# ThomasZiegler/RS-aware-differential-SfM

Measured on AMD Instinct MI355X. Metric: Mpixels/sec RS depth+pose solve, 1280x720 pair, higher is better.
Workload: dtype f64

## Files before the change

### include/rsdsfm.h

```cpp
#ifndef RSDSFM_H
#define RSDSFM_H

#include <stddef.h>
#include <stdint.h>

#ifdef __cplusplus
extern "C" {
#endif

#define RSDSFM_OK 0
#define RSDSFM_ERR_INVALID (-1)
#define RSDSFM_ERR_HIP (-2)
#define RSDSFM_ERR_NO_DEVICE (-3)
#define RSDSFM_ERR_NUMERIC (-4)
#define RSDSFM_ERR_PENDING (-5)
#define RSDSFM_ERR_PEER (-6)

#define RSDSFM_DEPTH_CLOSED_FORM 0
#define RSDSFM_DEPTH_CERES_LM 1

#define RSDSFM_K_COMPAT 0
#define RSDSFM_K_FIXED 1

#define RSDSFM_FLOW_COMPAT_RANK 0
// ... 152 lines not shown
    int32_t rows, cols;
    double fx, fy, cx, cy, gamma;
    double* d_depth_map_colmajor;
    double* d_R_rows9_or_null;
    double* d_t_rows3_or_null;
    uint64_t seed;
} rsdsfm_frame_job;
int rsdsfm_solve_frames_dev(rsdsfm_ctx* ctx, const rsdsfm_frame_job* jobs, int32_t count, const rsdsfm_frame_params* params,
                            rsdsfm_frame_result* results);
int rsdsfm_set_sequence_lanes(rsdsfm_ctx* ctx, int32_t lanes);
int rsdsfm_set_frame_side_flatten(rsdsfm_ctx* ctx, int mode);
int rsdsfm_set_frame_tail(rsdsfm_ctx* ctx, int mode);
int rsdsfm_set_frame_handoff(rsdsfm_ctx* ctx, int mode);
int rsdsfm_set_frame_predict(rsdsfm_ctx* ctx, int mode);
int rsdsfm_lma_predict_stats(rsdsfm_ctx* ctx, int64_t* hypotheses, int64_t* ended_where_predicted);
int rsdsfm_ransac_dev(rsdsfm_ctx* ctx, const double* d_q2n, const double* d_u2n, const double* d_alpha_n,
                      const double* d_alpha_k_n, int64_t n, int use_alpha_k, int32_t iterations, double tolerance,
                      const int32_t* samples_9xT_or_null, uint64_t seed, int depth_mode, int k_sign_mode,
                      rsdsfm_ransac_out* out);
int rsdsfm_refine_dev(rsdsfm_ctx* ctx, const double* d_flow2n, int64_t n_flow, int64_t m, const double* d_inliers_3m,
                      const double* d_alpha_m, const double* d_alpha_k_m, const int64_t* d_inlier_idx_or_null,
                      const double v_in[3], const double w_in[3], double k_in, int const_acceleration,
                      int flow_index_mode, double* d_inliers_out_3m, double v_out[3], double w_out[3], double* k_out,
                      rsdsfm_lm_summary* summary_or_null);
int rsdsfm_estimate_inverse_depths_batch_dev(rsdsfm_ctx* const* ctxs, int32_t count, const double* const* d_q2n,
                                             const double* const* d_u2n, const int64_t* n, const double* v_count_x3,
                                             const double* w_count_x3, const double* k_count, const double* const* d_alpha_n,
                                             const double* const* d_alpha_k_n, double* const* d_inv_depth_n);
int rsdsfm_depth_lm_batch_launch_dev(rsdsfm_ctx* const* ctxs, int32_t count, const double* const* d_q2n, const double* const* d_u2n,
                                     const int64_t* n, const double* v_count_x3, const double* w_count_x3, const double* k_count,
// ... 143 lines not shown
```

### rs-aware-differential-sfm_amd/__init__.py

```python
import contextlib
import ctypes as C
import os
import sys

import numpy as np

from . import dist, pipeline, synth

_HERE = os.path.dirname(os.path.abspath(__file__))
LIB_PATH = os.environ.get("RSDSFM_LIB") or os.path.join(_HERE, "librsdsfm_hip.so")
LIB_PATH_FUSED = os.path.join(_HERE, "librsdsfm_hip_fused.so")
HEADER_PATH = os.path.join(os.path.dirname(_HERE), "include", "rsdsfm.h")

OK = 0
ERR_PENDING = -5
DEPTH_CLOSED_FORM, DEPTH_CERES_LM = 0, 1
K_COMPAT, K_FIXED = 0, 1
FLOW_COMPAT_RANK, FLOW_GATHERED = 0, 1
REFINE_TRACE_COLS = 8
TRACE_REJECTED, TRACE_ACCEPTED, TRACE_INVALID, TRACE_PARAMETER_TOL, TRACE_FUNCTION_TOL, TRACE_ACCEPTED_GRADIENT_TOL = 0.0, 1.0, 2.0, 3.0, 4.0, 5.0
TERMINATION = {0: "gradient", 1: "parameter", 2: "function", 3: "max_iter", 4: "failure", 5: "min_radius"}

_libs = {}

# ... 491 lines not shown

    def set_sequence_lanes(self, lanes):
        self._check(self.lib.rsdsfm_set_sequence_lanes(self._ctx, C.c_int32(int(lanes))), "rsdsfm_set_sequence_lanes")

    def set_frame_side_flatten(self, on):
        self._check(self.lib.rsdsfm_set_frame_side_flatten(self._ctx, int(on)), "rsdsfm_set_frame_side_flatten")

    def set_frame_tail(self, mode):
        self._check(self.lib.rsdsfm_set_frame_tail(self._ctx, int(mode)), "rsdsfm_set_frame_tail")

    def set_frame_handoff(self, mode):
        self._check(self.lib.rsdsfm_set_frame_handoff(self._ctx, int(mode)), "rsdsfm_set_frame_handoff")

    def set_frame_predict(self, mode):
        self._check(self.lib.rsdsfm_set_frame_predict(self._ctx, int(mode)), "rsdsfm_set_frame_predict")

    def prepared_frames_solve(self, jobs, trials=50, tol=0.05, use_acceleration_mode=False, use_refinement=True, depth_mode=DEPTH_CERES_LM,
                              k_sign_mode=K_COMPAT, flow_threshold=1e-10, flow_index_mode=FLOW_COMPAT_RANK, use_global_shutter_mode=False):
        n = len(jobs)
        arr = (FrameJob * n)()
        for a, j in zip(arr, jobs):
            K = j["K"]
            a.d_flow_img, a.rows, a.cols = int(j["d_flow_img"]), int(j["rows"]), int(j["cols"])
            a.fx, a.fy, a.cx, a.cy, a.gamma = float(K[0]), float(K[1]), float(K[2]), float(K[3]), float(j["gamma"])
            a.d_depth_map, a.d_R, a.d_t = int(j["d_depth_map"]), int(j.get("d_R") or 0) or None, int(j.get("d_t") or 0) or None
        prm = FrameParams(int(trials), int(use_acceleration_mode), int(use_refinement), int(depth_mode), int(k_sign_mode),
                          int(flow_index_mode), int(use_global_shutter_mode), 0, float(tol), float(flow_threshold), 0)
        res = (FrameResult * n)()
        fn, ctx, check = self.lib.rsdsfm_solve_frames_dev, self._ctx, self._check

# ... 2053 lines not shown
```

### rs-aware-differential-sfm_amd/csrc/frame_host.hip

```cpp
#include <stdlib.h>
#include <string.h>

#include <atomic>

#include <algorithm>
#include <new>

#include "rsdsfm_internal.hpp"
#include "sequence_host.hpp"

namespace rsdsfm {

static std::atomic<int> g_frames_in_flight[64];
int frames_in_flight(const Ctx* c) { return g_frames_in_flight[c->device & 63].load(std::memory_order_relaxed); }

int alpha_ones_launch(Ctx* c, double* d_alpha, int64_t n);
int flatten_device(Ctx* c, const double* d_img, int32_t rows, int32_t cols, int32_t col0, double fx, double fy, double cx, double cy, double gamma,
                   double thr, double* d_q, double* d_u, double* d_alpha, double* d_alpha_k, int64_t* n_out);

struct FrameRun {
    rsdsfm_frame_job job;
    rsdsfm_frame_params prm;
    size_t N = 0;
    int64_t n = 0;
// ... 376 lines not shown
int rsdsfm_set_frame_handoff(rsdsfm_ctx* ctx, int mode) {
    if (!ctx) return RSDSFM_ERR_INVALID;
    if (mode < 0 || mode > 1) return fail(&ctx->c, RSDSFM_ERR_INVALID, "mode must be 0 (the first refinement pass gathers its inliers) or 1 (the compaction launch)");
    ctx->c.frame_handoff = mode;
    return RSDSFM_OK;
}

int rsdsfm_set_frame_predict(rsdsfm_ctx* ctx, int mode) {
    if (!ctx) return RSDSFM_ERR_INVALID;
    if (mode < 0 || mode > 2) return fail(&ctx->c, RSDSFM_ERR_INVALID, "mode must be 0 (the pixel pass fuses each hypothesis' predicted iterate), 1 (the two-iterate pass) or 2 (0 with the prediction inverted)");
    ctx->c.frame_predict = mode;
    for (rsdsfm_ctx* lane : ctx->c.lanes) lane->c.frame_predict = mode;
    return RSDSFM_OK;
}

int rsdsfm_set_frame_side_flatten(rsdsfm_ctx* ctx, int mode) {
    if (!ctx) return RSDSFM_ERR_INVALID;
    if (mode < 0 || mode > 3) return fail(&ctx->c, RSDSFM_ERR_INVALID, "mode must be 0 (flatten first), 1 (flatten on a second stream), 2 (flatten behind the minimal solver) or 3 (flatten inside the solver's launch)");
    ctx->c.frame_side_flatten = mode;
    return RSDSFM_OK;
}

}

namespace rsdsfm {

int sequence_lane_count(const Ctx* c, int count) { return std::max(1, std::min<int>(count, c->seq_lanes > 0 ? c->seq_lanes : kSequenceLanesDefault)); }

int solve_frames_run(Ctx* c, const rsdsfm_frame_job* jobs, int32_t count, const rsdsfm_frame_params* prm, rsdsfm_frame_result* results, const PairHook* hook) {
    const int L = sequence_lane_count(c, count);
// ... 8 lines not shown
        if (!c->ev_seq) RSDSFM_HIP_CHECK(c, hipEventCreateWithFlags(&c->ev_seq, hipEventDisableTiming));
        RSDSFM_HIP_CHECK(c, hipEventRecord(c->ev_seq, c->stream));
    }
    for (int l = 1; l < L; ++l) {
        Ctx* lc = lane_ctx(l);
        RSDSFM_HIP_CHECK(c, hipStreamWaitEvent(lc->stream, c->ev_seq, 0));
        lc->ransac_k0 = c->ransac_k0;
        lc->ransac_math_mode = c->ransac_math_mode;
        lc->lm_arithmetic = c->lm_arithmetic;
        lc->refine_arithmetic = c->refine_arithmetic;
        lc->lma_count_only_force = c->lma_count_only_force;
        lc->frame_side_flatten = c->frame_side_flatten;
        lc->frame_tail = c->frame_tail;
        lc->frame_handoff = c->frame_handoff;
        lc->frame_predict = c->frame_predict;
        lc->refine_stage_mode = c->refine_stage_mode;
    }
    for (int l = 0; l < L; ++l) lane_ctx(l)->refine_stage_separate = L > 1;
    int first_error = RSDSFM_OK;
    int in_flight[16];
    for (int l = 0; l < 16; ++l) in_flight[l] = -1;
    auto finish_lane = [&](int l) {
        const int i = in_flight[l];
        if (i < 0) return;
        in_flight[l] = -1;
        Ctx* lc = lane_ctx(l);
        int rc = frame_finish(lc, static_cast<FrameRun*>(lc->frame_run), &results[i]);
        if (rc != RSDSFM_OK && first_error == RSDSFM_OK) {
            first_error = rc;
            if (lc != c) c->err = "pair " + std::to_string(i) + ": " + lc->err;
// ... 63 lines not shown
```

### rs-aware-differential-sfm_amd/csrc/lma_common.hpp

```cpp
#pragma once

#include "device_math.hpp"
#include "lm_common.hpp"
#include "rsdsfm_internal.hpp"

namespace rsdsfm {

constexpr double kLmaHIrr = 1.01e-6;
constexpr double kLmaEta = 1e-11;
constexpr double kLmaMarginFloor = 128.0 * 0x1p-53;
constexpr double kLmaBand = 1e-6;
constexpr double kLmaSqrtMin = 0x1p-767;

constexpr int kLmaNC = 3;
constexpr int kLmaKP = 4;
constexpr int kLmaListCap = 1024;
constexpr int kLmaSlots = 6 + 2 * kLmaNC;
constexpr int kLmaG = 5;
constexpr int kLmaRowX0 = 8;
constexpr int kLmaRowXk = 10;
constexpr int kLmaRowScore = kLmaRowXk + 5 * kLmaKP;
constexpr int kLmaRow = kLmaRowScore + 2 * kLmaNC;

struct LmaPlan {
// ... 30 lines not shown
    int count_only;
    LmaPlan plan;
};

struct LmaPx {
    double a, ge, e0, rhos, h, g;
    bool clamped;
};

__device__ __forceinline__ double lma_max_pos(double x, double lo) {
    double r;
    asm("v_max_f64 %0, %1, %2" : "=v"(r) : "v"(x), "v"(lo));
    return r;
}
template <bool FULL = false>
__device__ __forceinline__ LmaPx lma_pixel(double x, double y, double ux, double uy, double al, double ak, const Pose& p, double two_over) {
    LmaPx o;
    const double beta = two_over * __builtin_fma(p.k, ak, al);
    const double a0 = __builtin_fma(x, p.v[2], -p.v[0]), a1 = __builtin_fma(y, p.v[2], -p.v[1]);
    const double J0 = beta * a0, J1 = beta * a1;
    const double xy = x * y, xx1 = __builtin_fma(x, x, 1.0), yy1 = __builtin_fma(y, y, 1.0);
    const double bw0 = __builtin_fma(xx1, p.w[1], __builtin_fma(-xy, p.w[0], -(y * p.w[2])));
    const double bw1 = __builtin_fma(xy, p.w[1], __builtin_fma(-yy1, p.w[0], x * p.w[2]));
    const double c0 = __builtin_fma(-beta, bw0, ux), c1 = __builtin_fma(-beta, bw1, uy);
    const double r0 = c0 + J0, r1 = c1 + J1;
    const double h = __builtin_fma(J0, J0, J1 * J1);
    double g = __builtin_fma(J0, r0, J1 * r1);
    const bool clamped = h < kLmaHIrr;
    g = g * __hiloint2double(clamped ? 0 : 0x3FF00000, 0);
    const double e0 = FULL ? g / lma_max_pos(h, kLmaHIrr) : div_core(g, lma_max_pos(h, kLmaHIrr));
    const double rhos = 1.0 - e0;
    const double s0 = __builtin_fma(rhos, J0, c0), s1 = __builtin_fma(rhos, J1, c1);
    o.a = __builtin_fma(s0, s0, s1 * s1);
    o.ge = g * e0;
    o.e0 = e0;
    o.rhos = rhos;
    o.h = h;
    o.g = g;
    o.clamped = clamped;
    return o;
}
__device__ __forceinline__ double lma_max_abs(double m, double x) {
    double r;
    asm("v_max_f64 %0, %1, |%2|" : "=v"(r) : "v"(m), "v"(x));
    return r;
}
__device__ __forceinline__ double lma_margin(const LmaPx& p, const LmaCand& cd) {
    const double t = (p.a + p.ge) + p.h;
    return __builtin_fma(t, cd.c1, cd.c1x2);
}
__device__ __forceinline__ void lma_score(const LmaPx& p, double phi2, double tol2, bool& in, double& err) {
    const double e2 = __builtin_fma(p.ge, phi2, p.a);
    in = e2 < tol2;
    err = (in && e2 >= kLmaSqrtMin) ? sqrt_core(e2) : 0.0;
}
// ... 48 lines not shown
```

### rs-aware-differential-sfm_amd/csrc/ransac_host.hip

```cpp
#include <stdio.h>
#include <stdlib.h>
#include <string.h>

#include <algorithm>
#include <vector>

#include "rsdsfm_internal.hpp"

namespace rsdsfm {

namespace {


inline uint64_t splitmix64(uint64_t& state) {
    uint64_t z = (state += 0x9E3779B97F4A7C15ULL);
    z = (z ^ (z >> 30)) * 0xBF58476D1CE4E5B9ULL;
    z = (z ^ (z >> 27)) * 0x94D049BB133111EBULL;
    return z ^ (z >> 31);
}

void sample_indices(int64_t n, int T, uint64_t seed, std::vector<int32_t>& out) {
    struct Slot {
        int64_t key;
        int32_t val;
// ... 124 lines not shown
                    R.round = 0;
                    R.pc = kPcRoundEnqueue;
                } else {
                    R.pc = kPcScore;
                }
                break;
            }
            case kPcRoundEnqueue: {
                const int b0 = R.b0, B = R.B, round = R.round;
                bool flags_via_pick = false;
                if (round > 4 * kMaxIter) return fail(c, RSDSFM_ERR_NUMERIC, "LM state machines did not terminate");
                if (R.analytic && round == 0) {
                    rc = ransac_lma_launch(c, R.d_q, R.d_u, R.d_a, R.d_ak, n, R.d_hyp + (size_t)b0 * 8, B, R.d_states + b0, R.d_partials, R.d_flags,
                                           R.d_scored + b0, R.d_tcount + b0, R.d_terr + b0, tol, R.lma_cand, 2, R.d_irr_count, R.d_irr_list, R.d_unscored,
                                           nullptr, R.core_epoch ? c->d_core_flag : nullptr, R.core_epoch, R.count_only,
                                           R.own_pass ? R.d_pred_steps + b0 : nullptr, reinterpret_cast<unsigned long long*>(c->d_core_flag + 4), c->frame_predict == 2);
                } else {
                    rc = ransac_lm_round_launch(c, R.d_q, R.d_u, R.d_a, R.d_ak, n, R.d_hyp + (size_t)b0 * 8, B, R.d_states + b0, R.d_partials, R.d_flags,
                                                R.d_scored + b0, R.d_tcount + b0, R.d_terr + b0, round, tol, R.k0, R.fused_base, R.core_math,
                                                R.core_epoch ? c->d_core_flag : nullptr, R.core_epoch, R.d_unscored);
                }
                if (rc != RSDSFM_OK) return rc;
                if (round == 0 && B == T) {
                    const PickLazy lazy = R.count_only ? PickLazy{R.d_scored, R.d_unscored, R.d_flags + 1} : PickLazy();
                    if (c->ransac_score_idle < kScoreIdleLimit) {
                        if (R.count_only) {
                            rc = ransac_pick_launch(c, R.d_tcount, R.d_terr, T, R.d_hyp, R.d_best, nullptr, R.d_flags, nullptr, 0, nullptr, 0, 0, nullptr, 0.0, lazy);
                            if (rc != RSDSFM_OK) return rc;
                        }
                        rc = ransac_score_launch(c, R.d_q, R.d_u, R.d_a, R.d_ak, n, R.d_hyp, T, R.d_states, depth_mode, tol, R.d_scored, R.d_partials,
                                                 R.d_tcount, R.d_terr, R.d_unscored, R.d_flags + 1);
// ... 417 lines not shown
```

### rs-aware-differential-sfm_amd/csrc/ransac_lma_kernels.hip

```cpp
#include <stdlib.h>

#include <algorithm>

#include "lma_common.hpp"
#include "lma_stages.hpp"
#include "rsdsfm_internal.hpp"

namespace rsdsfm {

namespace {

__device__ __forceinline__ bool is_nan_bits2(double x) {
    const uint32_t h = (uint32_t)__double2hiint(x) & 0x7FFFFFFFu;
    return h > 0x7FF00000u || (h == 0x7FF00000u && __double2loint(x) != 0);
}
__device__ __forceinline__ Pose load_pose(const double* __restrict__ hyp, int t) {
    const double* h_ = hyp + (int64_t)t * 8;
    Pose p;
    p.w[0] = h_[0], p.w[1] = h_[1], p.w[2] = h_[2];
    p.v[0] = h_[3], p.v[1] = h_[4], p.v[2] = h_[5];
    p.k = h_[6];
    return p;
}
__device__ __forceinline__ bool pose_nan(const Pose& p) {
    return is_nan_bits2(p.w[0]) || is_nan_bits2(p.w[1]) || is_nan_bits2(p.w[2]) || is_nan_bits2(p.v[0]) || is_nan_bits2(p.v[1]) || is_nan_bits2(p.v[2]) ||
           is_nan_bits2(p.k);
}

}

__device__ __forceinline__ int lma_own_index(const LmaCand& cd, int pred) { return pred == cd.steps[1] ? 1 : 0; }

template <int NC, bool ERR, bool OWN>
__device__ __forceinline__ void lma_pass_body(const double2* __restrict__ q, const double2* __restrict__ u, const double* __restrict__ alpha,
                                              const double* __restrict__ alpha_k, int64_t n, const double* __restrict__ hyp, int T, const LmaCand& cd,
                                              double* __restrict__ partials, int* __restrict__ irr_count, int* __restrict__ irr_list, int64_t chunk,
                                              unsigned long long* __restrict__ clk_probe, int clk_bid, int Tg, int nwg, const int* __restrict__ pred_steps) {
    static_assert(!OWN || NC == 1, "the own-iterate form fuses one iterate");
    __shared__ double s_part[kLB][kLmaSlots + 1];
    const int g = threadIdx.x;
    if ((int)blockIdx.x == clk_bid && g == 0) {
        clk_probe[0] = __builtin_amdgcn_s_memtime();
        clk_probe[1] = __builtin_amdgcn_s_memrealtime();
    }
    const int grp = (int)blockIdx.x / nwg, bid = (int)blockIdx.x - grp * nwg;
    const int t0 = grp * Tg, Tl = min(Tg, T - t0);
    const int P = kLB / Tg;
    const int slot = g / Tg, tl = g - slot * Tg, t = t0 + tl;
    const bool active = slot < P && tl < Tl;
    const int64_t p0 = (int64_t)bid * chunk;
    const int len = (int)min(chunk, n - p0);
    const double2* __restrict__ qb = q + p0;
    const double2* __restrict__ ub = u + p0;
    const double* __restrict__ ab = alpha + p0;
    const double* __restrict__ akb = alpha_k + p0;
    double A = 0.0, B = 0.0, C = 0.0, D = 0.0, E = 0.0, G = 0.0;
    int cnt[NC];
    double es[NC];
#pragma unroll
    for (int c = 0; c < NC; ++c) cnt[c] = 0, es[c] = 0.0;
    if (active) {
        const Pose pose = load_pose(hyp, t);
        const double two_over = 2.0 / (2.0 + pose.k);
        const double phi2_own = OWN ? (lma_own_index(cd, pred_steps[t]) ? cd.phi2[1] : cd.phi2[0]) : 0.0;
        auto pixel = [&](const PixIn& px) -> bool {
            const LmaPx v = lma_pixel(px.x, px.y, px.ux, px.uy, px.al, px.ak, pose, two_over);
            A += v.a;
            B += v.ge;
            C = __builtin_fma(v.e0, v.e0, C);
            D = __builtin_fma(v.rhos, v.rhos, D);
            E = __builtin_fma(v.rhos, v.e0, E);
            G = lma_max_abs(G, v.g);
            const double m = lma_margin(v, cd);
            bool listed = v.clamped;
#pragma unroll
            for (int c = 0; c < NC; ++c) {
                const double e2 = __builtin_fma(v.ge, OWN ? phi2_own : cd.phi2[c], v.a);
                const bool in = e2 < cd.tol2;
                listed = listed || (fabs(e2 - cd.tol2) <= m);
                cnt[c] += in ? 1 : 0;
                if (ERR) {
                    const double err = sqrt_core(lma_max_pos(e2, kLmaSqrtMin));
                    es[c] = __builtin_fma(err, __hiloint2double((in && e2 >= kLmaSqrtMin) ? 0x3FF00000 : 0, 0), es[c]);
                }
            }
            return listed;
        };
        auto push = [&](unsigned i) {
            const int pos = atomicAdd(&irr_count[t], 1);
            if (pos < kLmaListCap) irr_list[(int64_t)t * kLmaListCap + pos] = (int)(p0 + (int64_t)i);
        };
        const int rounds = len / P;
        unsigned i = (unsigned)slot;
        const unsigned uP = (unsigned)P;
        PixIn pa, pb;
        int r = 0;
        if (rounds > 0) pa = load_pix(qb, ub, ab, akb, i);
        for (; r + 1 < rounds; r += 2, i += 2 * uP) {
            pb = load_pix(qb, ub, ab, akb, i + uP);
            const bool la = pixel(pa);
            pa = load_pix(qb, ub, ab, akb, r + 2 < rounds ? i + 2 * uP : i);
            const bool lb = pixel(pb);
            if (la || lb) {
                if (la) push(i);
                if (lb) push(i + uP);
            }
        }
        if (r < rounds) {
            if (pixel(pa)) push(i);
            i += uP;
        }
        if (i < (unsigned)len && pixel(load_pix(qb, ub, ab, akb, i))) push(i);
    }
    s_part[g][0] = A, s_part[g][1] = B, s_part[g][2] = C, s_part[g][3] = D, s_part[g][4] = E, s_part[g][kLmaG] = G;
#pragma unroll
    for (int c = 0; c < kLmaNC; ++c) {
        s_part[g][6 + 2 * c] = c < NC ? (double)cnt[c < NC ? c : 0] : 0.0;
        s_part[g][7 + 2 * c] = c < NC ? es[c < NC ? c : 0] : 0.0;
    }
    __syncthreads();
    for (int o = g; o < Tl * kLmaSlots; o += kLB) {
        const int tt = o / kLmaSlots, sl = o - tt * kLmaSlots;
        double r = s_part[tt][sl];
        for (int s = 1; s < P; ++s) r = sl == kLmaG ? fmax(r, s_part[s * Tg + tt][sl]) : r + s_part[s * Tg + tt][sl];
        partials[((int64_t)(t0 + tt) * nwg + bid) * kLmaSlots + sl] = r;
    }
    if ((int)blockIdx.x == clk_bid && g == 0) {
        clk_probe[2] = __builtin_amdgcn_s_memtime();
        clk_probe[3] = __builtin_amdgcn_s_memrealtime();
    }
}

template <int NC, bool ERR>
__global__ __launch_bounds__(kLB) __attribute__((amdgpu_waves_per_eu(4, 5))) void ransac_lma_kernel(const double2* __restrict__ q, const double2* __restrict__ u, const double* __restrict__ alpha,
                                                        const double* __restrict__ alpha_k, int64_t n, const double* __restrict__ hyp, int T,
                                                        const LmaCand cd, double* __restrict__ partials, int* __restrict__ irr_count,
                                                        int* __restrict__ irr_list, int64_t chunk, unsigned long long* __restrict__ clk_probe, int clk_bid,
                                                        int Tg, int nwg) {
    lma_pass_body<NC, ERR, false>(q, u, alpha, alpha_k, n, hyp, T, cd, partials, irr_count, irr_list, chunk, clk_probe, clk_bid, Tg, nwg, nullptr);
}
template <bool ERR>
__global__ __launch_bounds__(kLB) __attribute__((amdgpu_waves_per_eu(4, 5))) void ransac_lma_own_kernel(const double2* __restrict__ q, const double2* __restrict__ u, const double* __restrict__ alpha,
                                                        const double* __restrict__ alpha_k, int64_t n, const double* __restrict__ hyp, int T,
                                                        const LmaCand cd, double* __restrict__ partials, int* __restrict__ irr_count,
                                                        int* __restrict__ irr_list, int64_t chunk, unsigned long long* __restrict__ clk_probe, int clk_bid,
                                                        int Tg, int nwg, const int* __restrict__ pred_steps) {
    lma_pass_body<1, ERR, true>(q, u, alpha, alpha_k, n, hyp, T, cd, partials, irr_count, irr_list, chunk, clk_probe, clk_bid, Tg, nwg, pred_steps);
}

__device__ __forceinline__ void lma_publish(int t, const LmScal& st, const double* hist_l, int fallback, bool scored, double count, double err,
                                            LmState* states, int* flags, int* __restrict__ scored_out, double* __restrict__ trial_count,
                                            double* __restrict__ trial_err, int* steps_hist, int* __restrict__ unscored_list, int* guard_word, bool count_only) {
    LmState* state = states + t;
    if (fallback) {
        LmScal f = {};
        f.status = 0;
        f.K = KMAX;
        f.termination = -1;
        f.rho_holds = -1;
        f.launches = 0;
        f.next_launch = 1;
        f.radius = kInitialRadius;
        f.decrease_factor = 2.0;
// ... 143 lines not shown
    }
    int64_t g = (n + (int64_t)P * 8 - 1) / ((int64_t)P * 8);
    g = std::max<int64_t>(1, std::min<int64_t>(g, (int64_t)c->num_cus * std::max(1, std::min(blocks_per_cu, 8))));
    int64_t chunk = (n + g - 1) / g;
    chunk = ((chunk + P - 1) / P) * P;
    g = std::max<int64_t>(1, (n + chunk - 1) / chunk);
    *chunk_out = chunk;
    return (int)g;
}
int64_t ransac_lma_partials_doubles(const Ctx* c, int64_t n, int batch) {
    const int64_t gmax = std::min<int64_t>((int64_t)c->num_cus * 8, std::max<int64_t>(1, (n + 7) / 8));
    return gmax * batch * kLmaSlots;
}
size_t ransac_lma_list_ints(int batch) { return (size_t)batch * kLmaListCap; }

static int lma_pass_launch(Ctx* c, const double* q, const double* u, const double* a, const double* ak, int64_t n, const double* hyp, int T,
                           const LmaCand& cd, double* partials, int* irr_count, int* irr_list, int* grid_out, unsigned long long* clk = nullptr,
                           const int* pred_steps = nullptr) {
    static int occ_tab[2][kLmaNC + 1] = {{0, 0, 0, 0}, {0, 0, 0, 0}};
    const int nc = pred_steps ? 0 : std::min(std::max(cd.nc, 1), (int)kLmaNC);
    int* occ = occ_tab[cd.count_only ? 1 : 0];
    if (occ[nc] == 0) {
        int nb = 0;
        const void* fn = pred_steps ? (cd.count_only ? reinterpret_cast<const void*>(&ransac_lma_own_kernel<false>) : reinterpret_cast<const void*>(&ransac_lma_own_kernel<true>))
                         : cd.count_only ? (nc == 1 ? reinterpret_cast<const void*>(&ransac_lma_kernel<1, false>) : nc == 2 ? reinterpret_cast<const void*>(&ransac_lma_kernel<2, false>) : reinterpret_cast<const void*>(&ransac_lma_kernel<3, false>))
                                       : (nc == 1 ? reinterpret_cast<const void*>(&ransac_lma_kernel<1, true>) : nc == 2 ? reinterpret_cast<const void*>(&ransac_lma_kernel<2, true>) : reinterpret_cast<const void*>(&ransac_lma_kernel<3, true>));
        if (hipOccupancyMaxActiveBlocksPerMultiprocessor(&nb, fn, kLB, 0) != hipSuccess || nb < 1) nb = 4;
        occ[nc] = nb;
    }
    int64_t chunk;
    static const int grid_override = getenv("RSDSFM_LMA_BLOCKS_PER_CU") ? atoi(getenv("RSDSFM_LMA_BLOCKS_PER_CU")) : 0;
    int groups = 1;
    const int Tg = ransac_lma_group_size(T, &groups);
    const int per_cu = std::max(1, (grid_override > 0 ? grid_override : occ[nc]));
    int nwg = ransac_lma_grid(c, n, Tg, &chunk, per_cu);
    if (groups > 1) {
        const int64_t cap = std::max<int64_t>(1, (int64_t)c->num_cus * std::min(per_cu, 8) / groups);
        if (nwg > cap) {
            const int P = std::max(1, kLB / Tg);
            chunk = (n + cap - 1) / cap;
            chunk = ((chunk + P - 1) / P) * P;
            nwg = (int)std::max<int64_t>(1, (n + chunk - 1) / chunk);
        }
    }
    const int grid = nwg * groups;
    *grid_out = nwg;
    const double2* q2 = reinterpret_cast<const double2*>(q);
    const double2* u2 = reinterpret_cast<const double2*>(u);
    const int clk_bid = clk ? grid / 2 : -1;
#define RSDSFM_LMA_LAUNCH(NC, ERR) \
    hipLaunchKernelGGL((ransac_lma_kernel<NC, ERR>), dim3(grid), dim3(kLB), 0, c->stream, q2, u2, a, ak, n, hyp, T, cd, partials, irr_count, irr_list, chunk, clk, clk_bid, Tg, nwg)
    if (pred_steps) {
        if (cd.count_only)
            hipLaunchKernelGGL((ransac_lma_own_kernel<false>), dim3(grid), dim3(kLB), 0, c->stream, q2, u2, a, ak, n, hyp, T, cd, partials, irr_count, irr_list, chunk, clk, clk_bid, Tg, nwg, pred_steps);
        else
            hipLaunchKernelGGL((ransac_lma_own_kernel<true>), dim3(grid), dim3(kLB), 0, c->stream, q2, u2, a, ak, n, hyp, T, cd, partials, irr_count, irr_list, chunk, clk, clk_bid, Tg, nwg, pred_steps);
    } else if (cd.count_only) {
        if (cd.nc == 1) RSDSFM_LMA_LAUNCH(1, false);
        else if (cd.nc == 2) RSDSFM_LMA_LAUNCH(2, false);
        else RSDSFM_LMA_LAUNCH(3, false);
    } else if (cd.nc == 1) RSDSFM_LMA_LAUNCH(1, true);
    else if (cd.nc == 2) RSDSFM_LMA_LAUNCH(2, true);
    else RSDSFM_LMA_LAUNCH(3, true);
#undef RSDSFM_LMA_LAUNCH
    RSDSFM_HIP_CHECK(c, hipGetLastError());
    return RSDSFM_OK;
}

int ransac_lma_launch(Ctx* c, const double* q, const double* u, const double* a, const double* ak, int64_t n, const double* hyp, int T,
                      LmState* states, double* partials, int* flags, int* scored, double* trial_count, double* trial_err, double tol,
                      const int* cand_steps, int ncand, int* irr_count, int* irr_list, int* unscored_list, int* guard_word, const int* m9_core_flag,
                      int m9_core_epoch, bool count_only, const int* pred_steps, unsigned long long* pred_stats, bool pred_discard) {
    if (T < 1 || T > kLB) return fail(c, RSDSFM_ERR_INVALID, "hypothesis batch of the analytic pass exceeds 256");
    if (pred_steps && ncand != 2) return fail(c, RSDSFM_ERR_INVALID, "the own-iterate pass chooses between two candidate iterates");
    const LmaCand cd = lma_candidates(cand_steps, ncand, tol, count_only);
    int grid = 0;
    const bool prof = c->profile && c->ev_prof[0] && c->ev_prof[1];
    if (prof) RSDSFM_HIP_CHECK(c, hipEventRecord(c->ev_prof[0], c->stream));
    int rc = lma_pass_launch(c, q, u, a, ak, n, hyp, T, cd, partials, irr_count, irr_list, &grid, prof ? c->d_clk_probe : nullptr, pred_steps);
    if (rc != RSDSFM_OK) return rc;
    if (prof) {
        RSDSFM_HIP_CHECK(c, hipEventRecord(c->ev_prof[1], c->stream));
        c->prof_pending = true;
        c->prof_what = 0;
    }
    hipLaunchKernelGGL(ransac_lma_rows_decide_kernel, dim3(T), dim3(kLB), 0, c->stream, partials, grid, T, reinterpret_cast<const double2*>(q),
                       reinterpret_cast<const double2*>(u), a, ak, n, hyp, cd, irr_count, irr_list, states, flags, scored, trial_count, trial_err,
                       unscored_list, guard_word, m9_core_flag, m9_core_epoch, pred_steps, pred_stats, pred_discard ? 1 : 0);
    RSDSFM_HIP_CHECK(c, hipGetLastError());
    return RSDSFM_OK;
}

int ransac_lma_rows_doubles() { return kLmaRow; }
int ransac_lma_rows_launch(Ctx* c, const double* q, const double* u, const double* a, const double* ak, int64_t n, const double* hyp, int T,
// ... 23 lines not shown
```

### rs-aware-differential-sfm_amd/csrc/rsdsfm_internal.hpp

```cpp
#pragma once

#include <hip/hip_runtime.h>
#include <stdint.h>

#include <functional>
#include <string>
#include <vector>

#include "../../include/rsdsfm.h"

namespace rsdsfm {

constexpr int kMaxIter = 50;
constexpr int kRefineTraceCols = RSDSFM_REFINE_TRACE_COLS;
constexpr double kInitialRadius = 1e4;
constexpr double kMaxRadius = 1e16;
constexpr double kMinRadius = 1e-32;
constexpr double kMinRelDecrease = 1e-3;
constexpr double kMinLmDiag = 1e-6;
constexpr double kMaxLmDiag = 1e32;
constexpr double kFunctionTol = 1e-6;
constexpr double kGradientTol = 1e-10;
static_assert(kGradientTol < 1.0, "the indicator encoding of the gradient-maximum slots needs kGradientTol < 1");
constexpr double kParameterTol = 1e-8;
// ... 136 lines not shown
    void* link = nullptr;
    void* fuse = nullptr;
    void* last_frame = nullptr;
    void* rectify_dense = nullptr;
    unsigned* d_claim[3] = {nullptr, nullptr, nullptr};
    size_t claim_words[3] = {0, 0, 0};
    unsigned claim_epoch[3] = {0, 0, 0};
    void* dist = nullptr;
    void* frame_run = nullptr;
    hipStream_t aux_stream = nullptr;
    hipEvent_t ev_fork = nullptr, ev_join = nullptr, ev_seq = nullptr;
    int frame_side_flatten = 3;
    int frame_tail = 0;
    int frame_handoff = 0;
    int frame_predict = 0;
    unsigned long long* d_flat_counters = nullptr;
    int seq_lanes = 0;
    int refine_stage_mode = 0;
    bool refine_stage_separate = false;
    int refine_arithmetic = 0;
    int64_t refine_rf_runs = 0, refine_rf_restarts = 0, refine_rf_resolves = 0;
    int refine_rf_last_guard = 0;
    struct RansacCache {
        uint64_t tag = 0, stage_gen = 0;
        const double *d_u = nullptr, *d_inl = nullptr, *d_alpha = nullptr, *d_alpha_k = nullptr;
        const int64_t* d_idx = nullptr;
        int64_t n = 0, m = 0;
        const void* h_u = nullptr;
        double u_probe[16] = {0};
        double inl_probe[16] = {0};
// ... 187 lines not shown
int ransac_decide_rows_launch(Ctx* c, const double* rows_all, int nranks, int T, LmState* states, int64_t n_total, int round,
                              int* flags, int* scored, double* trial_count, double* trial_err, bool core_trailer = false,
                              double* cnt_rt = nullptr, int cnt_stride = 0);
int ransac_score_rows_launch(Ctx* c, const double* q, const double* u, const double* a, const double* ak, int64_t n,
                             const double* hyp, int T, const LmState* states, int depth_mode, double tol, const int* scored,
                             double* partials, double* rows);
int ransac_score_merge_launch(Ctx* c, const double* rows_all, int nranks, int T, const int* scored, double* trial_count,
                              double* trial_err, double* cnt_rt = nullptr, int cnt_stride = 0);
void sample_indices(int64_t n, int T, uint64_t seed, int32_t* out);
int64_t ransac_lma_partials_doubles(const Ctx* c, int64_t n, int batch);
size_t ransac_lma_list_ints(int batch);
int ransac_lma_launch(Ctx* c, const double* q, const double* u, const double* a, const double* ak, int64_t n, const double* hyp, int T,
                      LmState* states, double* partials, int* flags, int* scored, double* trial_count, double* trial_err, double tol,
                      const int* cand_steps, int ncand, int* irr_count, int* irr_list, int* unscored_list, int* guard_word,
                      const int* m9_core_flag = nullptr, int m9_core_epoch = 0, bool count_only = false, const int* pred_steps = nullptr,
                      unsigned long long* pred_stats = nullptr, bool pred_discard = false);
int ransac_lma_rows_doubles();
int ransac_lma_rows_launch(Ctx* c, const double* q, const double* u, const double* a, const double* ak, int64_t n, const double* hyp, int T,
                           double* partials, double tol, const int* cand_steps, int ncand, int* irr_count, int* irr_list, double* rows);
int ransac_lma_decide_rows_launch(Ctx* c, const double* rows_all, int nranks, int64_t rank_stride, int T, int64_t n_total, const double* hyp,
                                  LmState* states, int* flags, int* scored, double* trial_count, double* trial_err, double tol, const int* cand_steps,
                                  int ncand, int* unscored_list, int* guard_word, double* cnt_rt, int cnt_stride, const int* m9_core_flag = nullptr,
                                  int m9_core_epoch = 0);
}

namespace rsdsfm {
struct RefineState {
    int32_t np, cur, iteration, invalid_run, num_successful, num_unsuccessful, termination, solve_ok;
    double p[7], pc[7], sp[7], yp[7];
    double radius, decrease_factor, cost, initial_cost, x_norm, gmax, stepsq_p;
    int64_t m;
// ... 186 lines not shown
```

Baseline: 1910.

## Stage per-pixel LMA operands in shared memory once per workgroup

Adds staged variants of the analytic LM pixel pass. Each workgroup loads a tile of pixel operands once into double-buffered LDS and shares them across all hypothesis lanes, instead of every lane loading them from global memory. When k is uniform it also precomputes the per-pixel beta and coordinate products (xy, x²+1, y²+1). By default staging is on when the hypothesis group size is at least 16. It adds block-wide barriers and more LDS use, which may lower occupancy.

```diff
diff --git a/include/rsdsfm.h b/include/rsdsfm.h
--- a/include/rsdsfm.h
+++ b/include/rsdsfm.h
@@ -190,6 +190,7 @@
 int rsdsfm_set_frame_handoff(rsdsfm_ctx* ctx, int mode);
 int rsdsfm_set_frame_predict(rsdsfm_ctx* ctx, int mode);
 int rsdsfm_lma_predict_stats(rsdsfm_ctx* ctx, int64_t* hypotheses, int64_t* ended_where_predicted);
+int rsdsfm_set_lma_operands(rsdsfm_ctx* ctx, int mode);
 int rsdsfm_ransac_dev(rsdsfm_ctx* ctx, const double* d_q2n, const double* d_u2n, const double* d_alpha_n,
                       const double* d_alpha_k_n, int64_t n, int use_alpha_k, int32_t iterations, double tolerance,
                       const int32_t* samples_9xT_or_null, uint64_t seed, int depth_mode, int k_sign_mode,
diff --git a/rs-aware-differential-sfm_amd/__init__.py b/rs-aware-differential-sfm_amd/__init__.py
--- a/rs-aware-differential-sfm_amd/__init__.py
+++ b/rs-aware-differential-sfm_amd/__init__.py
@@ -529,6 +529,9 @@
 
     def set_frame_predict(self, mode):
         self._check(self.lib.rsdsfm_set_frame_predict(self._ctx, int(mode)), "rsdsfm_set_frame_predict")
+
+    def set_lma_operands(self, mode):
+        self._check(self.lib.rsdsfm_set_lma_operands(self._ctx, int(mode)), "rsdsfm_set_lma_operands")
 
     def prepared_frames_solve(self, jobs, trials=50, tol=0.05, use_acceleration_mode=False, use_refinement=True, depth_mode=DEPTH_CERES_LM,
                               k_sign_mode=K_COMPAT, flow_threshold=1e-10, flow_index_mode=FLOW_COMPAT_RANK, use_global_shutter_mode=False):
diff --git a/rs-aware-differential-sfm_amd/csrc/frame_host.hip b/rs-aware-differential-sfm_amd/csrc/frame_host.hip
--- a/rs-aware-differential-sfm_amd/csrc/frame_host.hip
+++ b/rs-aware-differential-sfm_amd/csrc/frame_host.hip
@@ -414,6 +414,14 @@
     return RSDSFM_OK;
 }
 
+int rsdsfm_set_lma_operands(rsdsfm_ctx* ctx, int mode) {
+    if (!ctx) return RSDSFM_ERR_INVALID;
+    if (mode < 0 || mode > 2) return fail(&ctx->c, RSDSFM_ERR_INVALID, "mode must be 0 (the pixel pass stages each pixel's operands once per workgroup), 1 (every lane loads its pixel's operands) or 2 (0 for every hypothesis count)");
+    ctx->c.lma_operands = mode;
+    for (rsdsfm_ctx* lane : ctx->c.lanes) lane->c.lma_operands = mode;
+    return RSDSFM_OK;
+}
+
 int rsdsfm_set_frame_side_flatten(rsdsfm_ctx* ctx, int mode) {
     if (!ctx) return RSDSFM_ERR_INVALID;
     if (mode < 0 || mode > 3) return fail(&ctx->c, RSDSFM_ERR_INVALID, "mode must be 0 (flatten first), 1 (flatten on a second stream), 2 (flatten behind the minimal solver) or 3 (flatten inside the solver's launch)");
@@ -452,6 +460,7 @@
         lc->frame_tail = c->frame_tail;
         lc->frame_handoff = c->frame_handoff;
         lc->frame_predict = c->frame_predict;
+        lc->lma_operands = c->lma_operands;
         lc->refine_stage_mode = c->refine_stage_mode;
     }
     for (int l = 0; l < L; ++l) lane_ctx(l)->refine_stage_separate = L > 1;
diff --git a/rs-aware-differential-sfm_amd/csrc/lma_common.hpp b/rs-aware-differential-sfm_amd/csrc/lma_common.hpp
--- a/rs-aware-differential-sfm_amd/csrc/lma_common.hpp
+++ b/rs-aware-differential-sfm_amd/csrc/lma_common.hpp
@@ -68,12 +68,10 @@
     return r;
 }
 template <bool FULL = false>
-__device__ __forceinline__ LmaPx lma_pixel(double x, double y, double ux, double uy, double al, double ak, const Pose& p, double two_over) {
+__device__ __forceinline__ LmaPx lma_pixel(double x, double y, double ux, double uy, double beta, double xy, double xx1, double yy1, const Pose& p) {
     LmaPx o;
-    const double beta = two_over * __builtin_fma(p.k, ak, al);
     const double a0 = __builtin_fma(x, p.v[2], -p.v[0]), a1 = __builtin_fma(y, p.v[2], -p.v[1]);
     const double J0 = beta * a0, J1 = beta * a1;
-    const double xy = x * y, xx1 = __builtin_fma(x, x, 1.0), yy1 = __builtin_fma(y, y, 1.0);
     const double bw0 = __builtin_fma(xx1, p.w[1], __builtin_fma(-xy, p.w[0], -(y * p.w[2])));
     const double bw1 = __builtin_fma(xy, p.w[1], __builtin_fma(-yy1, p.w[0], x * p.w[2]));
     const double c0 = __builtin_fma(-beta, bw0, ux), c1 = __builtin_fma(-beta, bw1, uy);
@@ -93,6 +91,16 @@
     o.g = g;
     o.clamped = clamped;
     return o;
+}
+__device__ __forceinline__ double lma_beta(double al, double ak, double k, double two_over) { return two_over * __builtin_fma(k, ak, al); }
+__device__ __forceinline__ void lma_products(double x, double y, double& xy, double& xx1, double& yy1) {
+    xy = x * y, xx1 = __builtin_fma(x, x, 1.0), yy1 = __builtin_fma(y, y, 1.0);
+}
+template <bool FULL = false>
+__device__ __forceinline__ LmaPx lma_pixel(double x, double y, double ux, double uy, double al, double ak, const Pose& p, double two_over) {
+    double xy, xx1, yy1;
+    lma_products(x, y, xy, xx1, yy1);
+    return lma_pixel<FULL>(x, y, ux, uy, lma_beta(al, ak, p.k, two_over), xy, xx1, yy1, p);
 }
 __device__ __forceinline__ double lma_max_abs(double m, double x) {
     double r;
diff --git a/rs-aware-differential-sfm_amd/csrc/ransac_host.hip b/rs-aware-differential-sfm_amd/csrc/ransac_host.hip
--- a/rs-aware-differential-sfm_amd/csrc/ransac_host.hip
+++ b/rs-aware-differential-sfm_amd/csrc/ransac_host.hip
@@ -162,7 +162,8 @@
                     rc = ransac_lma_launch(c, R.d_q, R.d_u, R.d_a, R.d_ak, n, R.d_hyp + (size_t)b0 * 8, B, R.d_states + b0, R.d_partials, R.d_flags,
                                            R.d_scored + b0, R.d_tcount + b0, R.d_terr + b0, tol, R.lma_cand, 2, R.d_irr_count, R.d_irr_list, R.d_unscored,
                                            nullptr, R.core_epoch ? c->d_core_flag : nullptr, R.core_epoch, R.count_only,
-                                           R.own_pass ? R.d_pred_steps + b0 : nullptr, reinterpret_cast<unsigned long long*>(c->d_core_flag + 4), c->frame_predict == 2);
+                                           R.own_pass ? R.d_pred_steps + b0 : nullptr, reinterpret_cast<unsigned long long*>(c->d_core_flag + 4), c->frame_predict == 2,
+                                           !R.use_alpha_k, 0.0);
                 } else {
                     rc = ransac_lm_round_launch(c, R.d_q, R.d_u, R.d_a, R.d_ak, n, R.d_hyp + (size_t)b0 * 8, B, R.d_states + b0, R.d_partials, R.d_flags,
                                                 R.d_scored + b0, R.d_tcount + b0, R.d_terr + b0, round, tol, R.k0, R.fused_base, R.core_math,
diff --git a/rs-aware-differential-sfm_amd/csrc/ransac_lma_kernels.hip b/rs-aware-differential-sfm_amd/csrc/ransac_lma_kernels.hip
--- a/rs-aware-differential-sfm_amd/csrc/ransac_lma_kernels.hip
+++ b/rs-aware-differential-sfm_amd/csrc/ransac_lma_kernels.hip
@@ -31,13 +31,66 @@
 
 __device__ __forceinline__ int lma_own_index(const LmaCand& cd, int pred) { return pred == cd.steps[1] ? 1 : 0; }
 
-template <int NC, bool ERR, bool OWN>
+enum { kLmaPerLane = 0, kLmaStageOperands = 1, kLmaStageProducts = 2, kLmaStageBeta = 3 };
+constexpr int kLmaTile = kLB;
+constexpr int kLmaStageMinT = 16;
+template <int STG>
+struct LmaStageDims {
+    static constexpr int head = STG == kLmaStageOperands ? 6 : 8;
+    static constexpr int rec = STG == kLmaStageProducts ? 9 : head;
+    static constexpr int buf = kLmaTile * rec;
+    static constexpr int part = kLB * (kLmaSlots + 1);
+    static constexpr int words = STG == kLmaPerLane ? part : (2 * buf > part ? 2 * buf : part);
+};
+struct LmaRec {
+    double2 a, b, c, d;
+    double e;
+};
+template <int STG>
+__device__ __forceinline__ void lma_stage_store(double* __restrict__ buf, int j, const PixIn& p, double k_uniform, double two_over_uniform) {
+    double2* __restrict__ h = reinterpret_cast<double2*>(buf) + j * (LmaStageDims<STG>::head / 2);
+    h[0] = make_double2(p.x, p.y);
+    h[1] = make_double2(p.ux, p.uy);
+    if (STG == kLmaStageOperands) {
+        h[2] = make_double2(p.al, p.ak);
+        return;
+    }
+    double xy, xx1, yy1;
+    lma_products(p.x, p.y, xy, xx1, yy1);
+    if (STG == kLmaStageProducts) {
+        h[2] = make_double2(p.al, p.ak);
+        h[3] = make_double2(xy, xx1);
+        buf[kLmaTile * 8 + j] = yy1;
+    } else {
+        h[2] = make_double2(lma_beta(p.al, p.ak, k_uniform, two_over_uniform), xy);
+        h[3] = make_double2(xx1, yy1);
+    }
+}
+template <int STG>
+__device__ __forceinline__ LmaRec lma_stage_read(const double* __restrict__ buf, int j) {
+    const double2* __restrict__ h = reinterpret_cast<const double2*>(buf) + j * (LmaStageDims<STG>::head / 2);
+    LmaRec r;
+    r.a = h[0], r.b = h[1], r.c = h[2];
+    r.d = STG == kLmaStageOperands ? make_double2(0.0, 0.0) : h[3];
+    r.e = STG == kLmaStageProducts ? buf[kLmaTile * 8 + j] : 0.0;
+    return r;
+}
+template <int STG>
+__device__ __forceinline__ LmaPx lma_stage_pixel(const LmaRec& r, const Pose& pose, double two_over) {
+    if (STG == kLmaStageOperands) return lma_pixel(r.a.x, r.a.y, r.b.x, r.b.y, r.c.x, r.c.y, pose, two_over);
+    if (STG == kLmaStageProducts) return lma_pixel(r.a.x, r.a.y, r.b.x, r.b.y, lma_beta(r.c.x, r.c.y, pose.k, two_over), r.d.x, r.d.y, r.e, pose);
+    return lma_pixel(r.a.x, r.a.y, r.b.x, r.b.y, r.c.x, r.c.y, r.d.x, r.d.y, pose);
+}
+
+template <int NC, bool ERR, bool OWN, int STG>
 __device__ __forceinline__ void lma_pass_body(const double2* __restrict__ q, const double2* __restrict__ u, const double* __restrict__ alpha,
                                               const double* __restrict__ alpha_k, int64_t n, const double* __restrict__ hyp, int T, const LmaCand& cd,
                                               double* __restrict__ partials, int* __restrict__ irr_count, int* __restrict__ irr_list, int64_t chunk,
-                                              unsigned long long* __restrict__ clk_probe, int clk_bid, int Tg, int nwg, const int* __restrict__ pred_steps) {
+                                              unsigned long long* __restrict__ clk_probe, int clk_bid, int Tg, int nwg, const int* __restrict__ pred_steps,
+                                              double k_uniform) {
     static_assert(!OWN || NC == 1, "the own-iterate form fuses one iterate");
-    __shared__ double s_part[kLB][kLmaSlots + 1];
+    __shared__ __attribute__((aligned(16))) double s_mem[LmaStageDims<STG>::words];
+    double(*s_part)[kLmaSlots + 1] = reinterpret_cast<double(*)[kLmaSlots + 1]>(s_mem);
     const int g = threadIdx.x;
     if ((int)blockIdx.x == clk_bid && g == 0) {
         clk_probe[0] = __builtin_amdgcn_s_memtime();
@@ -59,12 +112,12 @@
     double es[NC];
 #pragma unroll
     for (int c = 0; c < NC; ++c) cnt[c] = 0, es[c] = 0.0;
-    if (active) {
-        const Pose pose = load_pose(hyp, t);
+    if (active || STG != kLmaPerLane) {
+        Pose pose = {};
+        if (active) pose = load_pose(hyp, t);
         const double two_over = 2.0 / (2.0 + pose.k);
-        const double phi2_own = OWN ? (lma_own_index(cd, pred_steps[t]) ? cd.phi2[1] : cd.phi2[0]) : 0.0;
-        auto pixel = [&](const PixIn& px) -> bool {
-            const LmaPx v = lma_pixel(px.x, px.y, px.ux, px.uy, px.al, px.ak, pose, two_over);
+        const double phi2_own = OWN && active ? (lma_own_index(cd, pred_steps[t]) ? cd.phi2[1] : cd.phi2[0]) : 0.0;
+        auto sums = [&](const LmaPx& v) -> bool {
             A += v.a;
             B += v.ge;
             C = __builtin_fma(v.e0, v.e0, C);
@@ -90,27 +143,76 @@
             const int pos = atomicAdd(&irr_count[t], 1);
             if (pos < kLmaListCap) irr_list[(int64_t)t * kLmaListCap + pos] = (int)(p0 + (int64_t)i);
         };
-        const int rounds = len / P;
-        unsigned i = (unsigned)slot;
         const unsigned uP = (unsigned)P;
-        PixIn pa, pb;
-        int r = 0;
-        if (rounds > 0) pa = load_pix(qb, ub, ab, akb, i);
-        for (; r + 1 < rounds; r += 2, i += 2 * uP) {
-            pb = load_pix(qb, ub, ab, akb, i + uP);
-            const bool la = pixel(pa);
-            pa = load_pix(qb, ub, ab, akb, r + 2 < rounds ? i + 2 * uP : i);
-            const bool lb = pixel(pb);
-            if (la || lb) {
-                if (la) push(i);
-                if (lb) push(i + uP);
+        if constexpr (STG == kLmaPerLane) {
+            auto pixel = [&](const PixIn& px) -> bool { return sums(lma_pixel(px.x, px.y, px.ux, px.uy, px.al, px.ak, pose, two_over)); };
+            const int rounds = len / P;
+            unsigned i = (unsigned)slot;
+            PixIn pa, pb;
+            int r = 0;
+            if (rounds > 0) pa = load_pix(qb, ub, ab, akb, i);
+            for (; r + 1 < rounds; r += 2, i += 2 * uP) {
+                pb = load_pix(qb, ub, ab, akb, i + uP);
+                const bool la = pixel(pa);
+                pa = load_pix(qb, ub, ab, akb, r + 2 < rounds ? i + 2 * uP : i);
+                const bool lb = pixel(pb);
+                if (la || lb) {
+                    if (la) push(i);
+                    if (lb) push(i + uP);
+                }
             }
-        }
-        if (r < rounds) {
-            if (pixel(pa)) push(i);
-            i += uP;
-        }
-        if (i < (unsigned)len && pixel(load_pix(qb, ub, ab, akb, i))) push(i);
+            if (r < rounds) {
+                if (pixel(pa)) push(i);
+                i += uP;
+            }
+            if (i < (unsigned)len && pixel(load_pix(qb, ub, ab, akb, i))) push(i);
+        } else {
+            constexpr int BUF = LmaStageDims<STG>::buf;
+            const int R0 = kLmaTile / P, R = R0 > 1 ? (R0 & ~1) : 1;
+            const int tile = R * P;
+            const int ntiles = (len + tile - 1) / tile;
+            const double two_over_uniform = 2.0 / (2.0 + k_uniform);
+            auto pixel = [&](const LmaRec& rc) -> bool { return sums(lma_stage_pixel<STG>(rc, pose, two_over)); };
+            PixIn sp = {};
+            if (g < min(tile, len)) {
+                sp = load_pix(qb, ub, ab, akb, (unsigned)g);
+                lma_stage_store<STG>(s_mem, g, sp, k_uniform, two_over_uniform);
+            }
+            for (int k = 0; k < ntiles; ++k) {
+                __syncthreads();
+                const int base = k * tile, m = min(tile, len - base);
+                const bool stage = g < min(tile, len - base - tile);
+                if (stage) sp = load_pix(qb, ub, ab, akb, (unsigned)(base + tile + g));
+                if (active) {
+                    const double* __restrict__ cur = s_mem + (k & 1) * BUF;
+                    const int rounds = m / P;
+                    unsigned j = (unsigned)slot;
+                    LmaRec pa, pb;
+                    int r = 0;
+                    constexpr bool CARRY = !(ERR && NC >= 2);
+                    if (CARRY && rounds > 0) pa = lma_stage_read<STG>(cur, j);
+                    for (; r + 1 < rounds; r += 2, j += 2 * uP) {
+                        if (!CARRY) pa = lma_stage_read<STG>(cur, j);
+                        pb = lma_stage_read<STG>(cur, j + uP);
+                        const bool la = pixel(pa);
+                        if (CARRY) pa = lma_stage_read<STG>(cur, r + 2 < rounds ? j + 2 * uP : j);
+                        const bool lb = pixel(pb);
+                        if (la || lb) {
+                            if (la) push((unsigned)base + j);
+                            if (lb) push((unsigned)base + j + uP);
+                        }
+                    }
+                    if (r < rounds) {
+                        if (!CARRY) pa = lma_stage_read<STG>(cur, j);
+                        if (pixel(pa)) push((unsigned)base + j);
+                        j += uP;
+                    }
+                    if (j < (unsigned)m && pixel(lma_stage_read<STG>(cur, j))) push((unsigned)base + j);
+                }
+                if (stage) lma_stage_store<STG>(s_mem + ((k + 1) & 1) * BUF, g, sp, k_uniform, two_over_uniform);
+            }
+            __syncthreads();
+        }
     }
     s_part[g][0] = A, s_part[g][1] = B, s_part[g][2] = C, s_part[g][3] = D, s_part[g][4] = E, s_part[g][kLmaG] = G;
 #pragma unroll
@@ -131,22 +233,30 @@
     }
 }
 
+#define RSDSFM_LMA_PASS_PARAMS                                                                                                                        \
+    const double2 *__restrict__ q, const double2 *__restrict__ u, const double *__restrict__ alpha, const double *__restrict__ alpha_k, int64_t n,     \
+        const double *__restrict__ hyp, int T, const LmaCand cd, double *__restrict__ partials, int *__restrict__ irr_count, int *__restrict__ irr_list, \
+        int64_t chunk, unsigned long long *__restrict__ clk_probe, int clk_bid, int Tg, int nwg
+#define RSDSFM_LMA_PASS_ARGS q, u, alpha, alpha_k, n, hyp, T, cd, partials, irr_count, irr_list, chunk, clk_probe, clk_bid, Tg, nwg
 template <int NC, bool ERR>
-__global__ __launch_bounds__(kLB) __attribute__((amdgpu_waves_per_eu(4, 5))) void ransac_lma_kernel(const double2* __restrict__ q, const double2* __restrict__ u, const double* __restrict__ alpha,
-                                                        const double* __restrict__ alpha_k, int64_t n, const double* __restrict__ hyp, int T,
-                                                        const LmaCand cd, double* __restrict__ partials, int* __restrict__ irr_count,
-                                                        int* __restrict__ irr_list, int64_t chunk, unsigned long long* __restrict__ clk_probe, int clk_bid,
-                                                        int Tg, int nwg) {
-    lma_pass_body<NC, ERR, false>(q, u, alpha, alpha_k, n, hyp, T, cd, partials, irr_count, irr_list, chunk, clk_probe, clk_bid, Tg, nwg, nullptr);
+__global__ __launch_bounds__(kLB) __attribute__((amdgpu_waves_per_eu(4, 5))) void ransac_lma_kernel(RSDSFM_LMA_PASS_PARAMS) {
+    lma_pass_body<NC, ERR, false, kLmaPerLane>(RSDSFM_LMA_PASS_ARGS, nullptr, 0.0);
 }
 template <bool ERR>
-__global__ __launch_bounds__(kLB) __attribute__((amdgpu_waves_per_eu(4, 5))) void ransac_lma_own_kernel(const double2* __restrict__ q, const double2* __restrict__ u, const double* __restrict__ alpha,
-                                                        const double* __restrict__ alpha_k, int64_t n, const double* __restrict__ hyp, int T,
-                                                        const LmaCand cd, double* __restrict__ partials, int* __restrict__ irr_count,
-                                                        int* __restrict__ irr_list, int64_t chunk, unsigned long long* __restrict__ clk_probe, int clk_bid,
-                                                        int Tg, int nwg, const int* __restrict__ pred_steps) {
-    lma_pass_body<1, ERR, true>(q, u, alpha, alpha_k, n, hyp, T, cd, partials, irr_count, irr_list, chunk, clk_probe, clk_bid, Tg, nwg, pred_steps);
-}
+__global__ __launch_bounds__(kLB) __attribute__((amdgpu_waves_per_eu(4, 5))) void ransac_lma_own_kernel(RSDSFM_LMA_PASS_PARAMS, const int* __restrict__ pred_steps) {
+    lma_pass_body<1, ERR, true, kLmaPerLane>(RSDSFM_LMA_PASS_ARGS, pred_steps, 0.0);
+}
+template <int NC, bool ERR, int STG>
+__global__ __launch_bounds__(kLB) __attribute__((amdgpu_waves_per_eu(4, 4))) void ransac_lma_staged_kernel(RSDSFM_LMA_PASS_PARAMS, double k_uniform) {
+    lma_pass_body<NC, ERR, false, STG>(RSDSFM_LMA_PASS_ARGS, nullptr, k_uniform);
+}
+template <bool ERR, int STG>
+__global__ __launch_bounds__(kLB) __attribute__((amdgpu_waves_per_eu(4, 4))) void ransac_lma_staged_own_kernel(RSDSFM_LMA_PASS_PARAMS, const int* __restrict__ pred_steps,
+                                                                                                         double k_uniform) {
+    lma_pass_body<1, ERR, true, STG>(RSDSFM_LMA_PASS_ARGS, pred_steps, k_uniform);
+}
+#undef RSDSFM_LMA_PASS_PARAMS
+#undef RSDSFM_LMA_PASS_ARGS
 
 __device__ __forceinline__ void lma_publish(int t, const LmScal& st, const double* hist_l, int fallback, bool scored, double count, double err,
                                             LmState* states, int* flags, int* __restrict__ scored_out, double* __restrict__ trial_count,
@@ -320,25 +430,51 @@
 }
 size_t ransac_lma_list_ints(int batch) { return (size_t)batch * kLmaListCap; }
 
+template <int STG>
+static const void* lma_pass_kernel(bool own, bool count_only, int nc) {
+#define RSDSFM_FN(...) reinterpret_cast<const void*>(&__VA_ARGS__)
+    if constexpr (STG == kLmaPerLane) {
+        if (own) return count_only ? RSDSFM_FN(ransac_lma_own_kernel<false>) : RSDSFM_FN(ransac_lma_own_kernel<true>);
+        if (count_only) return nc == 1 ? RSDSFM_FN(ransac_lma_kernel<1, false>) : nc == 2 ? RSDSFM_FN(ransac_lma_kernel<2, false>) : RSDSFM_FN(ransac_lma_kernel<3, false>);
+        return nc == 1 ? RSDSFM_FN(ransac_lma_kernel<1, true>) : nc == 2 ? RSDSFM_FN(ransac_lma_kernel<2, true>) : RSDSFM_FN(ransac_lma_kernel<3, true>);
+    } else {
+        if (own) return count_only ? RSDSFM_FN(ransac_lma_staged_own_kernel<false, STG>) : RSDSFM_FN(ransac_lma_staged_own_kernel<true, STG>);
+        if constexpr (STG == kLmaStageOperands) return nullptr;
+        else {
+            if (count_only)
+                return nc == 1 ? RSDSFM_FN(ransac_lma_staged_kernel<1, false, STG>) : nc == 2 ? RSDSFM_FN(ransac_lma_staged_kernel<2, false, STG>) : RSDSFM_FN(ransac_lma_staged_kernel<3, false, STG>);
+            return nc == 1 ? RSDSFM_FN(ransac_lma_staged_kernel<1, true, STG>) : nc == 2 ? RSDSFM_FN(ransac_lma_staged_kernel<2, true, STG>) : RSDSFM_FN(ransac_lma_staged_kernel<3, true, STG>);
+        }
+    }
+#undef RSDSFM_FN
+}
+
 static int lma_pass_launch(Ctx* c, const double* q, const double* u, const double* a, const double* ak, int64_t n, const double* hyp, int T,
                            const LmaCand& cd, double* partials, int* irr_count, int* irr_list, int* grid_out, unsigned long long* clk = nullptr,
-                           const int* pred_steps = nullptr) {
-    static int occ_tab[2][kLmaNC + 1] = {{0, 0, 0, 0}, {0, 0, 0, 0}};
-    const int nc = pred_steps ? 0 : std::min(std::max(cd.nc, 1), (int)kLmaNC);
-    int* occ = occ_tab[cd.count_only ? 1 : 0];
-    if (occ[nc] == 0) {
+                           const int* pred_steps = nullptr, bool k_uniform = false, double k_value = 0.0) {
+    const bool own = pred_steps != nullptr;
+    const int nc = std::min(std::max(cd.nc, 1), (int)kLmaNC);
+    static const int stage_override = getenv("RSDSFM_LMA_STAGE") ? atoi(getenv("RSDSFM_LMA_STAGE")) : -1;
+    int groups = 1;
+    int Tg = ransac_lma_group_size(T, &groups);
+    const bool staged = stage_override != 0 && (c->lma_operands == 2 || (c->lma_operands == 0 && Tg >= kLmaStageMinT));
+    int stg = !staged ? kLmaPerLane : k_uniform ? kLmaStageBeta : kLmaStageProducts;
+    if (stg != kLmaPerLane && stage_override == 2) stg = kLmaStageProducts;
+    if (stg != kLmaPerLane && stage_override == 1 && own) stg = kLmaStageOperands;
+    const void* fn = stg == kLmaPerLane         ? lma_pass_kernel<kLmaPerLane>(own, cd.count_only != 0, nc)
+                     : stg == kLmaStageOperands ? lma_pass_kernel<kLmaStageOperands>(own, cd.count_only != 0, nc)
+                     : stg == kLmaStageProducts ? lma_pass_kernel<kLmaStageProducts>(own, cd.count_only != 0, nc)
+                                                : lma_pass_kernel<kLmaStageBeta>(own, cd.count_only != 0, nc);
+    static int occ_tab[4][2][kLmaNC + 1] = {};
+    int& occ = occ_tab[stg][cd.count_only ? 1 : 0][own ? 0 : nc];
+    if (occ == 0) {
         int nb = 0;
-        const void* fn = pred_steps ? (cd.count_only ? reinterpret_cast<const void*>(&ransac_lma_own_kernel<false>) : reinterpret_cast<const void*>(&ransac_lma_own_kernel<true>))
-                         : cd.count_only ? (nc == 1 ? reinterpret_cast<const void*>(&ransac_lma_kernel<1, false>) : nc == 2 ? reinterpret_cast<const void*>(&ransac_lma_kernel<2, false>) : reinterpret_cast<const void*>(&ransac_lma_kernel<3, false>))
-                                       : (nc == 1 ? reinterpret_cast<const void*>(&ransac_lma_kernel<1, true>) : nc == 2 ? reinterpret_cast<const void*>(&ransac_lma_kernel<2, true>) : reinterpret_cast<const void*>(&ransac_lma_kernel<3, true>));
         if (hipOccupancyMaxActiveBlocksPerMultiprocessor(&nb, fn, kLB, 0) != hipSuccess || nb < 1) nb = 4;
-        occ[nc] = nb;
+        occ = nb;
     }
     int64_t chunk;
     static const int grid_override = getenv("RSDSFM_LMA_BLOCKS_PER_CU") ? atoi(getenv("RSDSFM_LMA_BLOCKS_PER_CU")) : 0;
-    int groups = 1;
-    const int Tg = ransac_lma_group_size(T, &groups);
-    const int per_cu = std::max(1, (grid_override > 0 ? grid_override : occ[nc]));
+    const int per_cu = std::max(1, (grid_override > 0 ? grid_override : occ));
     int nwg = ransac_lma_grid(c, n, Tg, &chunk, per_cu);
     if (groups > 1) {
         const int64_t cap = std::max<int64_t>(1, (int64_t)c->num_cus * std::min(per_cu, 8) / groups);
@@ -353,22 +489,13 @@
     *grid_out = nwg;
     const double2* q2 = reinterpret_cast<const double2*>(q);
     const double2* u2 = reinterpret_cast<const double2*>(u);
-    const int clk_bid = clk ? grid / 2 : -1;
-#define RSDSFM_LMA_LAUNCH(NC, ERR) \
-    hipLaunchKernelGGL((ransac_lma_kernel<NC, ERR>), dim3(grid), dim3(kLB), 0, c->stream, q2, u2, a, ak, n, hyp, T, cd, partials, irr_count, irr_list, chunk, clk, clk_bid, Tg, nwg)
-    if (pred_steps) {
-        if (cd.count_only)
-            hipLaunchKernelGGL((ransac_lma_own_kernel<false>), dim3(grid), dim3(kLB), 0, c->stream, q2, u2, a, ak, n, hyp, T, cd, partials, irr_count, irr_list, chunk, clk, clk_bid, Tg, nwg, pred_steps);
-        else
-            hipLaunchKernelGGL((ransac_lma_own_kernel<true>), dim3(grid), dim3(kLB), 0, c->stream, q2, u2, a, ak, n, hyp, T, cd, partials, irr_count, irr_list, chunk, clk, clk_bid, Tg, nwg, pred_steps);
-    } else if (cd.count_only) {
-        if (cd.nc == 1) RSDSFM_LMA_LAUNCH(1, false);
-        else if (cd.nc == 2) RSDSFM_LMA_LAUNCH(2, false);
-        else RSDSFM_LMA_LAUNCH(3, false);
-    } else if (cd.nc == 1) RSDSFM_LMA_LAUNCH(1, true);
-    else if (cd.nc == 2) RSDSFM_LMA_LAUNCH(2, true);
-    else RSDSFM_LMA_LAUNCH(3, true);
-#undef RSDSFM_LMA_LAUNCH
+    int clk_bid = clk ? grid / 2 : -1;
+    LmaCand cdv = cd;
+    void* args[18] = {&q2, &u2, &a, &ak, &n, &hyp, &T, &cdv, &partials, &irr_count, &irr_list, &chunk, &clk, &clk_bid, &Tg, &nwg, nullptr, nullptr};
+    int na = 16;
+    if (own) args[na++] = &pred_steps;
+    if (stg != kLmaPerLane) args[na++] = &k_value;
+    RSDSFM_HIP_CHECK(c, hipLaunchKernel(fn, dim3(grid), dim3(kLB), args, 0, c->stream));
     RSDSFM_HIP_CHECK(c, hipGetLastError());
     return RSDSFM_OK;
 }
@@ -376,14 +503,15 @@
 int ransac_lma_launch(Ctx* c, const double* q, const double* u, const double* a, const double* ak, int64_t n, const double* hyp, int T,
                       LmState* states, double* partials, int* flags, int* scored, double* trial_count, double* trial_err, double tol,
                       const int* cand_steps, int ncand, int* irr_count, int* irr_list, int* unscored_list, int* guard_word, const int* m9_core_flag,
-                      int m9_core_epoch, bool count_only, const int* pred_steps, unsigned long long* pred_stats, bool pred_discard) {
+                      int m9_core_epoch, bool count_only, const int* pred_steps, unsigned long long* pred_stats, bool pred_discard, bool k_uniform,
+                      double k_value) {
     if (T < 1 || T > kLB) return fail(c, RSDSFM_ERR_INVALID, "hypothesis batch of the analytic pass exceeds 256");
     if (pred_steps && ncand != 2) return fail(c, RSDSFM_ERR_INVALID, "the own-iterate pass chooses between two candidate iterates");
     const LmaCand cd = lma_candidates(cand_steps, ncand, tol, count_only);
     int grid = 0;
     const bool prof = c->profile && c->ev_prof[0] && c->ev_prof[1];
     if (prof) RSDSFM_HIP_CHECK(c, hipEventRecord(c->ev_prof[0], c->stream));
-    int rc = lma_pass_launch(c, q, u, a, ak, n, hyp, T, cd, partials, irr_count, irr_list, &grid, prof ? c->d_clk_probe : nullptr, pred_steps);
+    int rc = lma_pass_launch(c, q, u, a, ak, n, hyp, T, cd, partials, irr_count, irr_list, &grid, prof ? c->d_clk_probe : nullptr, pred_steps, k_uniform, k_value);
     if (rc != RSDSFM_OK) return rc;
     if (prof) {
         RSDSFM_HIP_CHECK(c, hipEventRecord(c->ev_prof[1], c->stream));
diff --git a/rs-aware-differential-sfm_amd/csrc/rsdsfm_internal.hpp b/rs-aware-differential-sfm_amd/csrc/rsdsfm_internal.hpp
--- a/rs-aware-differential-sfm_amd/csrc/rsdsfm_internal.hpp
+++ b/rs-aware-differential-sfm_amd/csrc/rsdsfm_internal.hpp
@@ -174,6 +174,7 @@
     int frame_tail = 0;
     int frame_handoff = 0;
     int frame_predict = 0;
+    int lma_operands = 0;
     unsigned long long* d_flat_counters = nullptr;
     int seq_lanes = 0;
     int refine_stage_mode = 0;
@@ -391,7 +392,8 @@
                       LmState* states, double* partials, int* flags, int* scored, double* trial_count, double* trial_err, double tol,
                       const int* cand_steps, int ncand, int* irr_count, int* irr_list, int* unscored_list, int* guard_word,
                       const int* m9_core_flag = nullptr, int m9_core_epoch = 0, bool count_only = false, const int* pred_steps = nullptr,
-                      unsigned long long* pred_stats = nullptr, bool pred_discard = false);
+                      unsigned long long* pred_stats = nullptr, bool pred_discard = false,
+                      bool k_uniform = false, double k_value = 0.0);
 int ransac_lma_rows_doubles();
 int ransac_lma_rows_launch(Ctx* c, const double* q, const double* u, const double* a, const double* ak, int64_t n, const double* hyp, int T,
                            double* partials, double tol, const int* cand_steps, int ncand, int* irr_count, int* irr_list, double* rows);
```

After: 1949, median of 6. +2.1%, better.
